# arnab39/Semi-supervised-segmentation-cycleGAN

Hardware: AMD Instinct MI355X
Metric: training images/sec (G+D step) at 256x256 (higher is better)
Workload: dtype f32; 1 GPU; VOC2012 21-class 256x256 semisupervised_cycleGAN as-written G+D step, batch=8 per GPU, fp32 tensors, 3-piece split-bf16 contraction, fp32-accurate (six exact bf16 piece products per fp32 product on the bf16 matrix cores, fp32 accumulation - forward, data and weight gradients; 21 / 20-channel stems and heads zero-padded onto the same contraction, 1- / 3-channel ends on the exact fp32 MFMA); global_batch=8, image_unit=one labeled + one unlabeled 256x256 image, parallelism=dp1, losses_finite=True

## Files before the change

semi-supervised-segmentation-cyclegan_amd/csrc/conv_wgrad.hip:

```cpp
#include "common.h"
#include <cstdlib>
#include "sscg_internal.h"

namespace {

constexpr int BKP = 32;

struct WgParams {
    const void* __restrict__ x;
    const void* __restrict__ dy;
    float* __restrict__ out;
    int Kc;
    int Ng;
    int C;
    int H, W, P, Q;
    int S;
    int stride, pad, dil, pad_mode;
    int npix;
    int chunk;
    int tiles_n;
    int tiles;
    int splits;
    float beta;
    FastDiv div_pq, div_q;
};

__device__ float sscg_zero_page[64];

template <int WM, int WN, int TM, int TN, int VA, int VB, bool DMA = false, int BF16 = 0, typename TX = float, typename TY = float>
__global__ __launch_bounds__(256) void conv_wgrad_kernel(WgParams p) {
    static_assert(!DMA || (VA == 4 && VB == 4), "LDS-DMA staging needs 16-byte granules");
    static_assert(!DMA || (sizeof(TX) == 4 && sizeof(TY) == 4), "LDS-DMA copies fp32 tiles");
    constexpr int BM = WM * TM * 32;
    constexpr int BN = WN * TN * 32;
    constexpr int LDA = DMA ? BM : BM + 4;
    constexpr int LDB = DMA ? BN : BN + 4;
    constexpr int CA = BM / VA;
    constexpr int CB = BN / VB;
    constexpr int RA = 256 / CA;
    constexpr int RB = 256 / CB;
    constexpr int PA = BKP / RA;
    constexpr int PB = BKP / RB;
    static_assert(256 % CA == 0 && 256 % CB == 0 && BKP % RA == 0 && BKP % RB == 0, "loader geometry");

    extern __shared__ __attribute__((aligned(16))) char smem_raw[];
    float* As = reinterpret_cast<float*>(smem_raw);
    float* Bs = As + 2 * BKP * LDA;

    const int tid = threadIdx.x;
    const int lin = xcd_remap(blockIdx.x, gridDim.x);
    const int split = lin / p.tiles;
    const int tl = lin - split * p.tiles;
    const int tile_n = tl % p.tiles_n;
    const int tile_m = tl / p.tiles_n;
    const int m0 = tile_m * BM;
    const int n0 = tile_n * BN;
    const int p_begin = split * p.chunk;
    const int p_end = min(p.npix, p_begin + p.chunk);

    const int ca = tid % CA, ra0 = tid / CA;
    const int ma = m0 + ca * VA;
    const bool a_col_ok = ma < p.Kc;
    const int cb = tid % CB, rb0 = tid / CB;
    const int nb = n0 + cb * VB;
    const bool b_col_ok = nb < p.Ng;
    int tdy = 0, tdx = 0, cch = 0;
    if (b_col_ok) {
        int tap = nb / p.C;
        cch = nb - tap * p.C;
        int ky = tap / p.S;
        int kx = tap - ky * p.S;
        tdy = ky * p.dil - p.pad;
        tdx = kx * p.dil - p.pad;
    }

    float ra[PA][VA];
    float rb[PB][VB];
    unsigned okmask = 0;

    const TY* dyc = reinterpret_cast<const TY*>(p.dy) + (a_col_ok ? ma : 0);
    const TX* xc = reinterpret_cast<const TX*>(p.x) + cch;
    const bool reflect = p.pad_mode == 1;

    int dma_buf = 0;
    const int wave_id = tid >> 6;
    auto load_tile = [&](int pt) {
        okmask = 0;
        if constexpr (DMA) {
            float* la = As + dma_buf * BKP * LDA + wave_id * 256;
            float* lb = Bs + dma_buf * BKP * LDB + wave_id * 256;
#pragma unroll
            for (int ps = 0; ps < PA; ++ps) {
                const int pix = pt + ra0 + ps * RA;
                const bool ok = a_col_ok && pix < p_end;
                const void* g = ok ? (const void*)(dyc + (size_t)pix * p.Kc) : (const void*)sscg_zero_page;
                __builtin_amdgcn_global_load_lds((const __attribute__((address_space(1))) void*)g,
                                                 (__attribute__((address_space(3))) void*)(la + ps * RA * LDA), 16, 0, 0);
            }
#pragma unroll
            for (int ps = 0; ps < PB; ++ps) {
                const int pix = pt + rb0 + ps * RB;
                bool ok = b_col_ok && pix < p_end;
                const int pp = ok ? pix : 0;
                const int img = fd_div(pp, p.div_pq);
                const int rem = pp - img * (p.P * p.Q);
                const int oy = fd_div(rem, p.div_q);
                const int ox = rem - oy * p.Q;
                int sy = oy * p.stride + tdy;
                int sx = ox * p.stride + tdx;
                int ry = sy < 0 ? -sy : sy;
                int rx = sx < 0 ? -sx : sx;
                ry = ry >= p.H ? 2 * (p.H - 1) - ry : ry;
                rx = rx >= p.W ? 2 * (p.W - 1) - rx : rx;
                sy = reflect ? ry : sy;
                sx = reflect ? rx : sx;
                ok = ok && ((unsigned)sy < (unsigned)p.H) && ((unsigned)sx < (unsigned)p.W);
                const void* g = ok ? (const void*)(xc + (size_t)((img * p.H + sy) * p.W + sx) * p.C) : (const void*)sscg_zero_page;
                __builtin_amdgcn_global_load_lds((const __attribute__((address_space(1))) void*)g,
                                                 (__attribute__((address_space(3))) void*)(lb + ps * RB * LDB), 16, 0, 0);
            }
            dma_buf ^= 1;
            return;
        }
#pragma unroll
        for (int ps = 0; ps < PA; ++ps) {
            const int pix = pt + ra0 + ps * RA;
            const bool ok = a_col_ok && pix < p_end;
            okmask |= ok ? (1u << ps) : 0u;
            const TY* g = dyc + (size_t)(ok ? pix : 0) * p.Kc;
            if constexpr (VA == 4) ld4<TY>(g, ra[ps]);
            else ra[ps][0] = ld1<TY>(g);
        }
#pragma unroll
        for (int ps = 0; ps < PB; ++ps) {
            const int pix = pt + rb0 + ps * RB;
            bool ok = b_col_ok && pix < p_end;
            const int pp = ok ? pix : 0;
            const int img = fd_div(pp, p.div_pq);
            const int rem = pp - img * (p.P * p.Q);
            const int oy = fd_div(rem, p.div_q);
            const int ox = rem - oy * p.Q;
            int sy = oy * p.stride + tdy;
            int sx = ox * p.stride + tdx;
            int ry = sy < 0 ? -sy : sy;
            int rx = sx < 0 ? -sx : sx;
            ry = ry >= p.H ? 2 * (p.H - 1) - ry : ry;
            rx = rx >= p.W ? 2 * (p.W - 1) - rx : rx;
            sy = reflect ? ry : sy;
            sx = reflect ? rx : sx;
            ok = ok && ((unsigned)sy < (unsigned)p.H) && ((unsigned)sx < (unsigned)p.W);
            okmask |= ok ? (1u << (16 + ps)) : 0u;
            const int spix = ok ? (img * p.H + sy) * p.W + sx : 0;
            const TX* g = xc + (size_t)spix * p.C;
            if constexpr (VB == 4) ld4<TX>(g, rb[ps]);
            else rb[ps][0] = ld1<TX>(g);
        }
    };

    auto store_tile = [&](int buf) {
        if constexpr (DMA) return;
        float* a = As + buf * BKP * LDA;
        float* b = Bs + buf * BKP * LDB;
#pragma unroll
        for (int ps = 0; ps < PA; ++ps) {
            float* d = a + (ra0 + ps * RA) * LDA + ca * VA;
            const bool ok = (okmask >> ps) & 1u;
            if constexpr (VA == 4) {
                f32x4 v;
#pragma unroll
                for (int e = 0; e < 4; ++e) v[e] = ok ? ra[ps][e] : 0.f;
                *reinterpret_cast<f32x4*>(d) = v;
            } else {
                *d = ok ? ra[ps][0] : 0.f;
            }
        }
#pragma unroll
        for (int ps = 0; ps < PB; ++ps) {
            float* d = b + (rb0 + ps * RB) * LDB + cb * VB;
            const bool ok = (okmask >> (16 + ps)) & 1u;
            if constexpr (VB == 4) {
                f32x4 v;
#pragma unroll
                for (int e = 0; e < 4; ++e) v[e] = ok ? rb[ps][e] : 0.f;
                *reinterpret_cast<f32x4*>(d) = v;
            } else {
                *d = ok ? rb[ps][0] : 0.f;
            }
        }
    };

    const int wave = tid >> 6;
    const int lane = tid & 63;
    const int li = lane & 31;
    const int lh = lane >> 5;
    const int wm = wave / WN;
    const int wn = wave % WN;
    const int row_w = wm * TM * 32;
    const int col_w = wn * TN * 32;

    f32x16 acc[TM][TN];
#pragma unroll
    for (int i = 0; i < TM; ++i)
#pragma unroll
        for (int j = 0; j < TN; ++j)
#pragma unroll
            for (int e = 0; e < 16; ++e) acc[i][j][e] = 0.f;

    const int nsteps = (p_end - p_begin + BKP - 1) / BKP;
    if (nsteps > 0) {
        load_tile(p_begin);
        store_tile(0);
    }
    __syncthreads();
    for (int it = 0; it < nsteps; ++it) {
        const int buf = it & 1;
        if (it + 1 < nsteps) load_tile(p_begin + (it + 1) * BKP);
        const float* a = As + buf * BKP * LDA + lh * LDA + row_w + li;
        const float* b = Bs + buf * BKP * LDB + lh * LDB + col_w + li;
        if constexpr (BF16) {
#pragma unroll
            for (int g2 = 0; g2 < BKP / 16; ++g2) {
                if constexpr (BF16 == 2) {
                    bf16x8 a0[TM], a1[TM], a2[TM], b0[TN], b1[TN], b2[TN];
#pragma unroll
                    for (int i = 0; i < TM; ++i) {
                        float v[8];
#pragma unroll
                        for (int e = 0; e < 8; ++e) v[e] = a[(g2 * 8 + e) * 2 * LDA + i * 32];
                        sscg_split8(v, a0[i], a1[i], a2[i]);
                    }
#pragma unroll
                    for (int j = 0; j < TN; ++j) {
                        float v[8];
#pragma unroll
                        for (int e = 0; e < 8; ++e) v[e] = b[(g2 * 8 + e) * 2 * LDB + j * 32];
                        sscg_split8(v, b0[j], b1[j], b2[j]);
                    }
#pragma unroll
                    for (int t = 0; t < 6; ++t)
#pragma unroll
                        for (int i = 0; i < TM; ++i)
#pragma unroll
                            for (int j = 0; j < TN; ++j) {
                                const bf16x8& pa = t == 0 ? a2[i] : (t == 1 || t == 3) ? a1[i] : a0[i];
                                const bf16x8& pb = (t == 0 || t == 3 || t == 5) ? b0[j] : (t == 1 || t == 4) ? b1[j] : b2[j];
                                acc[i][j] = __builtin_amdgcn_mfma_f32_32x32x16_bf16(pa, pb, acc[i][j], 0, 0, 0);
                            }
                    continue;
                }
                bf16x8 pa[TM], pb[TN];
#pragma unroll
                for (int e = 0; e < 8; ++e) {
                    const int kp = g2 * 8 + e;
#pragma unroll
                    for (int i = 0; i < TM; ++i) pa[i][e] = (__bf16)a[kp * 2 * LDA + i * 32];
#pragma unroll
                    for (int j = 0; j < TN; ++j) pb[j][e] = (__bf16)b[kp * 2 * LDB + j * 32];
                }
#pragma unroll
                for (int i = 0; i < TM; ++i)
#pragma unroll
                    for (int j = 0; j < TN; ++j)
                        acc[i][j] = __builtin_amdgcn_mfma_f32_32x32x16_bf16(pa[i], pb[j], acc[i][j], 0, 0, 0);
            }
        } else {
#pragma unroll
        for (int kp = 0; kp < BKP / 2; ++kp) {
            float fa[TM], fb[TN];
#pragma unroll
            for (int i = 0; i < TM; ++i) fa[i] = a[kp * 2 * LDA + i * 32];
#pragma unroll
            for (int j = 0; j < TN; ++j) fb[j] = b[kp * 2 * LDB + j * 32];
#pragma unroll
            for (int i = 0; i < TM; ++i)
#pragma unroll
                for (int j = 0; j < TN; ++j)
                    acc[i][j] = __builtin_amdgcn_mfma_f32_32x32x2f32(fa[i], fb[j], acc[i][j], 0, 0, 0);
        }
        }
        if (it + 1 < nsteps) store_tile(buf ^ 1);
        __syncthreads();
    }

    float* out = p.out + (size_t)split * p.Kc * p.Ng;
    const bool direct = (p.splits == 1);
    if constexpr (VB == 4) {
        sscg_stage_store_tile<BM, BN, 256, TM, TN>(acc, reinterpret_cast<float*>(smem_raw), out, m0, n0, p.Kc, p.Ng, row_w, col_w, li, lh, tid,
                                                   direct ? p.beta : 0.f);
        return;
    }
#pragma unroll
    for (int j = 0; j < TN; ++j) {
        const int n = n0 + col_w + j * 32 + li;
        if (n >= p.Ng) continue;
#pragma unroll
        for (int i = 0; i < TM; ++i) {
#pragma unroll
            for (int e = 0; e < 16; ++e) {
                const int m = m0 + row_w + i * 32 + (e & 3) + 8 * (e >> 2) + 4 * lh;
                if (m < p.Kc) {
                    size_t o = (size_t)m * p.Ng + n;
                    float v = acc[i][j][e];
                    if (direct && p.beta != 0.f) v += p.beta * out[o];
                    out[o] = v;
                }
            }
        }
    }
}

template <int V>
__global__ __launch_bounds__(256) void wgrad_reduce_kernel(const float* __restrict__ ws, float* __restrict__ dw, size_t n, int splits,
                                                            float beta) {
    const size_t i = ((size_t)blockIdx.x * blockDim.x + threadIdx.x) * V;
    if (i >= n) return;
    typedef float vec_t __attribute__((ext_vector_type(V)));
    vec_t s = 0.f;
#pragma unroll 16
    for (int k = 0; k < splits; ++k) s += *reinterpret_cast<const vec_t*>(ws + (size_t)k * n + i);
    vec_t* d = reinterpret_cast<vec_t*>(dw + i);
    *d = (beta != 0.f) ? beta * *d + s : s;
}

__global__ __launch_bounds__(256) void wgrad_reduce_w4_kernel(const float* __restrict__ ws, float* __restrict__ dw, size_t n, int splits,
                                                               float beta) {
    __shared__ f32x4 sm[3][64];
    const int v = threadIdx.x & 63, sl = threadIdx.x >> 6;
    const size_t i = ((size_t)blockIdx.x * 64 + v) * 4;
    f32x4 s = 0.f;
    if (i < n) {
#pragma unroll 8
        for (int k = sl; k < splits; k += 4) s += *reinterpret_cast<const f32x4*>(ws + (size_t)k * n + i);
    }
    if (sl) sm[sl - 1][v] = s;
    __syncthreads();
    if (sl == 0 && i < n) {
        s = ((s + sm[0][v]) + sm[1][v]) + sm[2][v];
        f32x4* d = reinterpret_cast<f32x4*>(dw + i);
        *d = (beta != 0.f) ? beta * *d + s : s;
    }
}

struct WgPlan {
    int cfg;
    int bm, bn;
    int splits;
    int chunk;
};


struct WgClass { int cfg, bm, bn; float t_step_us, c0; float f[4]; };
const WgClass WG_CLASSES[] = {
    {0, 128, 128, 2.13f, 1.5f, {1.25f, 1.f, 1.f, 1.f}},
    {1, 64, 64, 0.59f, 2.f, {1.5f, 1.17f, 1.08f, 1.f}},
    {2, 32, 128, 0.70f, 2.f, {1.5f, 1.17f, 1.08f, 1.f}},
    {3, 128, 32, 0.70f, 2.f, {1.5f, 1.17f, 1.08f, 1.f}},
};

float wgrad_cost_us(const WgClass& c, long tiles, long steps, long s, double out_bytes) {
    long r = cdiv(tiles * s, 256);
    float f = c.f[r > 4 ? 3 : r - 1];
    float t = (float)r * ((float)cdiv(steps, s) + c.c0) * c.t_step_us * f;
    if (s > 1) t += (float)(2.0 * s * out_bytes / 4.0e6) + 4.f;
    return t;
}

WgPlan plan_wgrad(const sscg_conv_desc* d) {
    WgPlan pl;
    const int Kc = d->K;
    const int Ng = d->R * d->S * d->C;
    const long npix = (long)d->N * d->P * d->Q;
    const long steps = cdiv(npix, BKP);
    const double out_bytes = (double)Kc * Ng * sizeof(float);
    int first = 0, last = 1;
    if (d->precision == 2 && Kc >= 128 && Ng >= 128) last = 0;
    if (Kc <= 32) first = last = 2;
    else if (Ng <= 32 || d->C < 32) first = last = 3;
    else if (Kc <= 64 || Ng <= 64) first = last = 1;
    float best = 0.f;
    long best_s = 1;
    pl.cfg = -1;
    for (int ci = first; ci <= last; ++ci) {
        const WgClass& c = WG_CLASSES[ci];
        const long tiles = (long)cdiv(Kc, c.bm) * cdiv(Ng, c.bn);
        const long smax = steps / 2 < 1 ? 1 : (steps / 2 > 512 ? 512 : steps / 2);
        long prev = 0;
        for (int k = 0; k <= 16; ++k) {
            long sp = k == 0 ? 1 : (256L * k) / tiles;
            if (sp < 1) sp = 1;
            if (sp > smax) sp = smax;
            if (sp == prev) continue;
            prev = sp;
            float t = wgrad_cost_us(c, tiles, steps, sp, out_bytes);
            if (pl.cfg < 0 || t < best) { best = t; best_s = sp; pl.cfg = c.cfg; pl.bm = c.bm; pl.bn = c.bn; }
        }
    }
    long splits = best_s;
    const int force_cfg = (d->wgrad_tuning & 0xff) - 1, force_splits = (d->wgrad_tuning >> 8) & 0xffff;
    if (force_cfg >= 0 && force_cfg <= 1 && force_splits > 0 && pl.cfg <= 1) {
        pl.cfg = force_cfg;
        pl.bm = pl.bn = pl.cfg == 0 ? 128 : 64;
        splits = force_splits;
        if (splits > steps) splits = steps;
    }
    long steps_per = cdiv(steps, splits);
    pl.chunk = (int)(steps_per * BKP);
    pl.splits = cdiv(npix, pl.chunk);
    return pl;
}

template <int WM, int WN, int TM, int TN, int VA, int VB, bool DMA = false, int BF16 = 0, typename TX = float, typename TY = float>
int launch_wg(WgParams p, int splits, hipStream_t st) {
    constexpr int BM = WM * TM * 32;
    constexpr int BN = WN * TN * 32;
    p.tiles_n = cdiv(p.Ng, BN);
    int tiles_m = cdiv(p.Kc, BM);
    p.tiles = tiles_m * p.tiles_n;
    p.splits = splits;
    size_t smem = (size_t)(2 * BKP * (DMA ? BM : BM + 4) + 2 * BKP * (DMA ? BN : BN + 4)) * sizeof(float);
    if (VB == 4 && smem < (size_t)BM * (BN + 4) * sizeof(float)) smem = (size_t)BM * (BN + 4) * sizeof(float);
    auto kern = conv_wgrad_kernel<WM, WN, TM, TN, VA, VB, DMA, BF16, TX, TY>;
    SSCG_ENSURE_SMEM((kern), smem);
    hipLaunchKernelGGL(kern, dim3(p.tiles * splits), dim3(256), smem, st, p);
    SSCG_LAUNCH_CHECK();
    return SSCG_OK;
}

template <int VA, int VB>
int dispatch_wg(const WgParams& p, const WgPlan& pl, int precision, hipStream_t st) {
    switch (pl.cfg) {
        case 0: if (precision == 1) return launch_wg<2, 2, 2, 2, VA, VB, (VA == 4 && VB == 4), 1>(p, pl.splits, st);
                if constexpr (VA == 4 && VB == 4) { if (precision == 2) return launch_wg<2, 2, 2, 2, VA, VB, true, 2>(p, pl.splits, st); }
                return launch_wg<2, 2, 2, 2, VA, VB, (VA == 4 && VB == 4)>(p, pl.splits, st);
        case 1: if (precision == 1) return launch_wg<2, 2, 1, 1, VA, VB, (VA == 4 && VB == 4), 1>(p, pl.splits, st);
                if constexpr (VA == 4 && VB == 4) { if (precision == 2) return launch_wg<2, 2, 1, 1, VA, VB, true, 2>(p, pl.splits, st); }
                return launch_wg<2, 2, 1, 1, VA, VB, (VA == 4 && VB == 4)>(p, pl.splits, st);
        case 2: if (precision == 1) return launch_wg<1, 4, 1, 1, VA, VB, false, true>(p, pl.splits, st);
                return launch_wg<1, 4, 1, 1, VA, VB>(p, pl.splits, st);
        case 3: if (precision == 1) return launch_wg<4, 1, 1, 1, VA, VB, false, true>(p, pl.splits, st);
                return launch_wg<4, 1, 1, 1, VA, VB>(p, pl.splits, st);
        default: return SSCG_ERR_BAD_ARG;
    }
}

template <int VA, int VB, typename TX, typename TY>
int dispatch_wg_mixed(const WgParams& p, const WgPlan& pl, hipStream_t st) {
    switch (pl.cfg) {
        case 2: return launch_wg<1, 4, 1, 1, VA, VB, false, true, TX, TY>(p, pl.splits, st);
        case 3: return launch_wg<4, 1, 1, 1, VA, VB, false, true, TX, TY>(p, pl.splits, st);
        default: return SSCG_ERR_UNSUPPORTED;
    }
}

template <typename TX, typename TY>
int dispatch_wg_types(const WgParams& p, const WgPlan& pl, bool va4, bool vb4, hipStream_t st) {
    if (va4 && vb4) return dispatch_wg_mixed<4, 4, TX, TY>(p, pl, st);
    if (va4) return dispatch_wg_mixed<4, 1, TX, TY>(p, pl, st);
    if (vb4) return dispatch_wg_mixed<1, 4, TX, TY>(p, pl, st);
    return dispatch_wg_mixed<1, 1, TX, TY>(p, pl, st);
}

}

namespace {

constexpr int THIN_MAX = 32;
constexpr int THIN_BLOCKS = 1024;

struct ThinParams {
    const void* __restrict__ wide;
    const void* __restrict__ thin;
    float* __restrict__ part;
    int npix, Wd, T;
};

template <int T, typename TW, typename TT>
__global__ __launch_bounds__(256) void thin_wgrad_kernel(ThinParams p) {
    const TW* wide = reinterpret_cast<const TW*>(p.wide);
    const TT* thin = reinterpret_cast<const TT*>(p.thin);
    constexpr int TB = T < 4 ? T : 4;
    extern __shared__ float red[];
    const int wq = p.Wd / 4;
    const int lanes = 256 / wq;
    const int q = threadIdx.x % wq;
    const int pl = threadIdx.x / wq;
    float acc[T][4];
#pragma unroll
    for (int t = 0; t < T; ++t)
#pragma unroll
        for (int e = 0; e < 4; ++e) acc[t][e] = 0.f;
    if (pl < lanes) {
        const int stride = lanes * gridDim.x;
        int px = blockIdx.x * lanes + pl;
        for (; px + stride < p.npix; px += 2 * stride) {
            float w0[4], w1[4];
            ld4<TW>(wide + (size_t)px * p.Wd + q * 4, w0);
            ld4<TW>(wide + (size_t)(px + stride) * p.Wd + q * 4, w1);
            const TT* th0 = thin + (size_t)px * T;
            const TT* th1 = thin + (size_t)(px + stride) * T;
#pragma unroll
            for (int t = 0; t < T; ++t) {
                const float v0 = ld1<TT>(th0 + t), v1 = ld1<TT>(th1 + t);
#pragma unroll
                for (int e = 0; e < 4; ++e) acc[t][e] = fmaf(v1, w1[e], fmaf(v0, w0[e], acc[t][e]));
            }
        }
        if (px < p.npix) {
            float w0[4];
            ld4<TW>(wide + (size_t)px * p.Wd + q * 4, w0);
            const TT* th0 = thin + (size_t)px * T;
#pragma unroll
            for (int t = 0; t < T; ++t) {
                const float v0 = ld1<TT>(th0 + t);
#pragma unroll
                for (int e = 0; e < 4; ++e) acc[t][e] = fmaf(v0, w0[e], acc[t][e]);
            }
        }
    }
#pragma unroll
    for (int t0 = 0; t0 < T; t0 += TB) {
        if (pl < lanes) {
#pragma unroll
            for (int t = 0; t < TB; ++t)
                if (t0 + t < T)
#pragma unroll
                    for (int e = 0; e < 4; ++e) red[((size_t)pl * TB + t) * p.Wd + q * 4 + e] = acc[t0 + t][e];
        }
        __syncthreads();
        const int nt = (T - t0) < TB ? (T - t0) : TB;
        for (int i = threadIdx.x; i < nt * p.Wd; i += 256) {
            float s = 0.f;
            for (int l = 0; l < lanes; ++l) s += red[(size_t)l * TB * p.Wd + i];
            p.part[(size_t)blockIdx.x * T * p.Wd + (size_t)t0 * p.Wd + i] = s;
        }
        __syncthreads();
    }
}

__global__ __launch_bounds__(256) void thin_wgrad_reduce_kernel(const float* __restrict__ part, float* __restrict__ dw, int blocks,
                                                                 int T, int Wd, int K, int C, float beta) {
    const int o = blockIdx.x * 4 + (threadIdx.x >> 6);
    const int lane = threadIdx.x & 63;
    if (o >= T * Wd) return;
    float s = 0.f;
    for (int b = lane; b < blocks; b += 64) s += part[(size_t)b * T * Wd + o];
    s = wave_sum(s);
    if (lane == 0) {
        const int t = o / Wd, w = o - t * Wd;
        const int k = (K == T && K <= C) ? t : w;
        const int c = (K == T && K <= C) ? w : t;
        float* d = dw + (size_t)k * C + c;
        *d = beta != 0.f ? beta * *d + s : s;
    }
}

bool thin_wgrad_applies(const sscg_conv_desc* d) {
    if (d->R != 1 || d->S != 1 || d->stride != 1 || d->pad != 0 || d->pad_mode != 0) return false;
    const int T = d->K < d->C ? d->K : d->C, Wd = d->K < d->C ? d->C : d->K;
    return T <= THIN_MAX && Wd % 4 == 0 && Wd <= 256 && Wd >= 16 && (long)d->N * d->H * d->W >= 65536;
}

template <int T, typename TW, typename TT>
int launch_thin(const ThinParams& p, int blocks, size_t smem, hipStream_t st) {
    SSCG_ENSURE_SMEM((thin_wgrad_kernel<T, TW, TT>), smem);
    hipLaunchKernelGGL((thin_wgrad_kernel<T, TW, TT>), dim3(blocks), dim3(256), smem, st, p);
    return SSCG_OK;
}

template <typename TW, typename TT>
int launch_thin_T(const ThinParams& p, size_t smem, hipStream_t st) {
    switch (p.T) {
        case 1: return launch_thin<1, TW, TT>(p, THIN_BLOCKS, smem, st);
        case 2: return launch_thin<2, TW, TT>(p, THIN_BLOCKS, smem, st);
        case 3: return launch_thin<3, TW, TT>(p, THIN_BLOCKS, smem, st);
        case 4: return launch_thin<4, TW, TT>(p, THIN_BLOCKS, smem, st);
        case 20: return launch_thin<20, TW, TT>(p, THIN_BLOCKS, smem, st);
        case 21: return launch_thin<21, TW, TT>(p, THIN_BLOCKS, smem, st);
        default: return SSCG_ERR_UNSUPPORTED;
    }
}

int thin_wgrad(const sscg_conv_desc* d, const void* x, const void* dy, float* dw, float beta, void* ws, hipStream_t st) {
    const bool thin_is_k = d->K <= d->C;
    ThinParams p;
    p.T = thin_is_k ? d->K : d->C;
    p.Wd = thin_is_k ? d->C : d->K;
    p.wide = thin_is_k ? x : dy;
    p.thin = thin_is_k ? dy : x;
    const int wide_dt = thin_is_k ? d->x_dtype : d->y_dtype, thin_dt = thin_is_k ? d->y_dtype : d->x_dtype;
    p.part = reinterpret_cast<float*>(ws);
    p.npix = d->N * d->H * d->W;
    const int lanes = 256 / (p.Wd / 4);
    const size_t smem = (size_t)lanes * (p.T < 4 ? p.T : 4) * p.Wd * sizeof(float);
    int rc;
    if (wide_dt == SSCG_F32 && thin_dt == SSCG_F32) rc = launch_thin_T<float, float>(p, smem, st);
    else if (wide_dt == SSCG_BF16 && thin_dt == SSCG_F32) rc = launch_thin_T<__bf16, float>(p, smem, st);
    else if (wide_dt == SSCG_BF16 && thin_dt == SSCG_BF16) rc = launch_thin_T<__bf16, __bf16>(p, smem, st);
    else rc = SSCG_ERR_UNSUPPORTED;
    if (rc) return rc;
    SSCG_LAUNCH_CHECK();
    hipLaunchKernelGGL(thin_wgrad_reduce_kernel, dim3(cdiv(p.T * p.Wd, 4)), dim3(256), 0, st, p.part, dw, THIN_BLOCKS, p.T, p.Wd,
                       d->K, d->C, beta);
    SSCG_LAUNCH_CHECK();
    return SSCG_OK;
}

bool thin_wgrad_supported_T(int T) { return T == 1 || T == 2 || T == 3 || T == 4 || T == 20 || T == 21; }

}

int sscg_wgrad_reduce(const float* ws, float* dw, size_t n, int splits, float beta, hipStream_t st) {
    static const bool w4 = !(getenv("SSCG_WGRAD_REDUCE_W4") && atoi(getenv("SSCG_WGRAD_REDUCE_W4")) == 0);
    const bool vec_ok = n % 4 == 0 && ((size_t)dw & 15) == 0 && ((size_t)ws & 15) == 0;
    if (vec_ok && w4 && splits >= 8 && n / 4 <= 64 * 16384)
        hipLaunchKernelGGL(wgrad_reduce_w4_kernel, dim3(cdiv((long)(n / 4), 64)), dim3(256), 0, st, ws, dw, n, splits, beta);
    else if (vec_ok)
        hipLaunchKernelGGL(wgrad_reduce_kernel<4>, dim3(cdiv((long)(n / 4), 256)), dim3(256), 0, st, ws, dw, n, splits, beta);
    else
        hipLaunchKernelGGL(wgrad_reduce_kernel<1>, dim3(cdiv((long)n, 256)), dim3(256), 0, st, ws, dw, n, splits, beta);
    SSCG_LAUNCH_CHECK();
    return SSCG_OK;
}

static bool wg_dt_ok(int dt) { return dt == SSCG_F32 || dt == SSCG_BF16; }

extern "C" size_t sscg_conv2d_wgrad_workspace(const sscg_conv_desc* d) {
    if (!d) return 0;
    if (thin_wgrad_applies(d) && thin_wgrad_supported_T(d->K < d->C ? d->K : d->C))
        return (size_t)THIN_BLOCKS * d->K * d->C * sizeof(float);
    if (sscg_wgrad16_applies(d)) return sscg_wgrad16_workspace(d);
    if (sscg_wgrads_applies(d)) return sscg_wgrads_workspace(d);
    WgPlan pl = plan_wgrad(d);
    if (pl.splits <= 1) return 0;
    return (size_t)pl.splits * d->K * d->R * d->S * d->C * sizeof(float);
}

extern "C" int sscg_conv2d_wgrad(const sscg_conv_desc* d, const void* x, const void* dy, float* dw, float beta,
                                 void* ws, size_t ws_bytes, void* stream) {
    if (!d || !x || !dy || !dw) return SSCG_ERR_BAD_ARG;
    if (d->N <= 0 || d->C <= 0 || d->K <= 0 || !wg_dt_ok(d->x_dtype) || !wg_dt_ok(d->y_dtype)) return SSCG_ERR_BAD_ARG;
    if ((long)d->N * d->H * d->W * (long)d->C >= (1L << 31)) return SSCG_ERR_UNSUPPORTED;
    if ((long)d->N * d->P * d->Q * (long)d->K >= (1L << 31)) return SSCG_ERR_UNSUPPORTED;
    hipStream_t st = (hipStream_t)stream;
    if (thin_wgrad_applies(d) && thin_wgrad_supported_T(d->K < d->C ? d->K : d->C)) {
        if (!ws || ws_bytes < sscg_conv2d_wgrad_workspace(d)) return SSCG_ERR_WORKSPACE;
        return thin_wgrad(d, x, dy, dw, beta, ws, st);
    }
    if (sscg_wgrad16_applies(d)) return sscg_wgrad16(d, x, dy, dw, beta, ws, ws_bytes, st);
    if (sscg_wgrads_applies(d)) return sscg_wgrads(d, x, dy, dw, beta, ws, ws_bytes, st);
    WgPlan pl = plan_wgrad(d);
    size_t need = pl.splits > 1 ? (size_t)pl.splits * d->K * d->R * d->S * d->C * sizeof(float) : 0;
    if (need > 0 && (!ws || ws_bytes < need)) return SSCG_ERR_WORKSPACE;
    WgParams p;
    p.x = x; p.dy = dy;
    p.out = pl.splits > 1 ? reinterpret_cast<float*>(ws) : dw;
    p.Kc = d->K; p.Ng = d->R * d->S * d->C; p.C = d->C;
    p.H = d->H; p.W = d->W; p.P = d->P; p.Q = d->Q; p.S = d->S;
    p.stride = d->stride; p.pad = d->pad; p.dil = d->dil; p.pad_mode = d->pad_mode;
    p.npix = d->N * d->P * d->Q; p.chunk = pl.chunk; p.tiles_n = 0; p.tiles = 0; p.splits = 1;
    p.beta = pl.splits > 1 ? 0.f : beta;
    p.div_pq = make_fastdiv(d->P * d->Q);
    p.div_q = make_fastdiv(d->Q);
    const bool va4 = (d->K % 4 == 0), vb4 = (d->C % 4 == 0);
    int rc;
    if (d->x_dtype == SSCG_F32 && d->y_dtype == SSCG_F32) {
        if (va4 && vb4) rc = dispatch_wg<4, 4>(p, pl, d->precision, st);
        else if (va4) rc = dispatch_wg<4, 1>(p, pl, d->precision, st);
        else if (vb4) rc = dispatch_wg<1, 4>(p, pl, d->precision, st);
        else rc = dispatch_wg<1, 1>(p, pl, d->precision, st);
    } else if (d->x_dtype == SSCG_F32) {
        rc = dispatch_wg_types<float, __bf16>(p, pl, va4, vb4, st);
    } else if (d->y_dtype == SSCG_F32) {
        rc = dispatch_wg_types<__bf16, float>(p, pl, va4, vb4, st);
    } else {
        rc = SSCG_ERR_UNSUPPORTED;
    }
    if (rc) return rc;
    if (pl.splits > 1) return sscg_wgrad_reduce(reinterpret_cast<const float*>(ws), dw, (size_t)d->K * p.Ng, pl.splits, beta, st);
    return SSCG_OK;
}
```

Measured before the change: 65.24 img/s.

## Add dedicated weight-gradient paths for thin and ragged-channel conv ends

```diff
diff --git a/semi-supervised-segmentation-cyclegan_amd/csrc/conv_wgrad.hip b/semi-supervised-segmentation-cyclegan_amd/csrc/conv_wgrad.hip
--- a/semi-supervised-segmentation-cyclegan_amd/csrc/conv_wgrad.hip
+++ b/semi-supervised-segmentation-cyclegan_amd/csrc/conv_wgrad.hip
@@ -427,7 +427,10 @@
 }
 
 template <int VA, int VB>
-int dispatch_wg(const WgParams& p, const WgPlan& pl, int precision, hipStream_t st) {
+int dispatch_wg(const WgParams& p, const WgPlan& pl, int precision, hipStream_t st, bool split_small = false) {
+    if constexpr (VA == 4 && VB == 4) {
+        if (split_small && precision == 2 && pl.cfg == 2) return launch_wg<1, 4, 1, 1, 4, 4, true, 2>(p, pl.splits, st);
+    }
     switch (pl.cfg) {
         case 0: if (precision == 1) return launch_wg<2, 2, 2, 2, VA, VB, (VA == 4 && VB == 4), 1>(p, pl.splits, st);
                 if constexpr (VA == 4 && VB == 4) { if (precision == 2) return launch_wg<2, 2, 2, 2, VA, VB, true, 2>(p, pl.splits, st); }
@@ -609,6 +612,175 @@
 
 }
 
+int sscg_wgrad_reduce(const float* ws, float* dw, size_t n, int splits, float beta, hipStream_t st);
+
+namespace {
+
+__global__ __launch_bounds__(256) void wgrad_reduce_cut_kernel(const float* __restrict__ ws, float* __restrict__ dw, size_t n_out, int C, int Cp,
+                                                                size_t split_stride, int splits, float beta) {
+    const size_t i = (size_t)blockIdx.x * 256 + threadIdx.x;
+    if (i >= n_out) return;
+    const size_t row = i / C;
+    const size_t src = row * Cp + (i - row * C);
+    float s = 0.f;
+#pragma unroll 8
+    for (int k = 0; k < splits; ++k) s += ws[(size_t)k * split_stride + src];
+    dw[i] = (beta != 0.f) ? beta * dw[i] + s : s;
+}
+
+constexpr int TT_SLAB = 256;
+constexpr int TT_MAXK = 3;
+
+struct ThinTapsParams {
+    const float* __restrict__ x;
+    const float* __restrict__ dy;
+    float* __restrict__ part;
+    int npix;
+    int H, W, C, P, Q, pad, dil;
+    int ppb;
+    FastDiv div_hw, div_w;
+};
+
+template <int T, int R, int S>
+__global__ __launch_bounds__(256) void thin_taps_wgrad_kernel(ThinTapsParams p) {
+    constexpr int TAPS = R * S;
+    __shared__ float red[4][TAPS][TT_SLAB];
+    const int lane = threadIdx.x & 63;
+    const int wv = __builtin_amdgcn_readfirstlane(threadIdx.x >> 6);
+    const int c0 = blockIdx.x * TT_SLAB + lane * 4;
+    const bool c_ok = c0 < p.C;
+    const int p0 = blockIdx.y * p.ppb;
+    const int p1 = min(p.npix, p0 + p.ppb);
+    float acc[T][TAPS][4];
+#pragma unroll
+    for (int t = 0; t < T; ++t)
+#pragma unroll
+        for (int k = 0; k < TAPS; ++k)
+#pragma unroll
+            for (int e = 0; e < 4; ++e) acc[t][k][e] = 0.f;
+    const float* xc = p.x + (c_ok ? c0 : 0);
+    f32x4 cur = 0.f;
+    int px = p0 + wv;
+    if (px < p1 && c_ok) cur = *reinterpret_cast<const f32x4*>(xc + (size_t)px * p.C);
+    for (; px < p1; px += 4) {
+        f32x4 nxt = 0.f;
+        if (px + 4 < p1 && c_ok) nxt = *reinterpret_cast<const f32x4*>(xc + (size_t)(px + 4) * p.C);
+        const int img = fd_div(px, p.div_hw);
+        const int rem = px - img * (p.H * p.W);
+        const int iy = fd_div(rem, p.div_w);
+        const int ix = rem - iy * p.W;
+#pragma unroll
+        for (int ky = 0; ky < R; ++ky) {
+            const int oy = iy + p.pad - ky * p.dil;
+            if ((unsigned)oy >= (unsigned)p.P) continue;
+#pragma unroll
+            for (int kx = 0; kx < S; ++kx) {
+                const int ox = ix + p.pad - kx * p.dil;
+                if ((unsigned)ox >= (unsigned)p.Q) continue;
+                const float* g = p.dy + (size_t)((img * p.P + oy) * p.Q + ox) * T;
+#pragma unroll
+                for (int t = 0; t < T; ++t) {
+                    const float v = g[t];
+#pragma unroll
+                    for (int e = 0; e < 4; ++e) acc[t][ky * S + kx][e] = fmaf(v, cur[e], acc[t][ky * S + kx][e]);
+                }
+            }
+        }
+        cur = nxt;
+    }
+#pragma unroll
+    for (int t = 0; t < T; ++t) {
+#pragma unroll
+        for (int k = 0; k < TAPS; ++k)
+            *reinterpret_cast<f32x4*>(&red[wv][k][lane * 4]) = f32x4{acc[t][k][0], acc[t][k][1], acc[t][k][2], acc[t][k][3]};
+        __syncthreads();
+        const int c = blockIdx.x * TT_SLAB + threadIdx.x;
+        if (c < p.C) {
+            float* o = p.part + ((size_t)blockIdx.y * T + t) * TAPS * p.C + c;
+#pragma unroll
+            for (int k = 0; k < TAPS; ++k)
+                o[(size_t)k * p.C] = ((red[0][k][threadIdx.x] + red[1][k][threadIdx.x]) + red[2][k][threadIdx.x]) + red[3][k][threadIdx.x];
+        }
+        __syncthreads();
+    }
+}
+
+struct EndsPlan {
+    int kind;
+    int Cp, Kp;
+    WgPlan pl;
+    size_t pad_bytes;
+    int ppb, pblocks;
+    size_t ws_bytes;
+};
+
+EndsPlan plan_ends(const sscg_conv_desc* d) {
+    static const bool on = !(getenv("SSCG_WGRAD_THIN_ENDS") && atoi(getenv("SSCG_WGRAD_THIN_ENDS")) == 0);
+    EndsPlan e;
+    e.kind = 0; e.Cp = d->C; e.Kp = d->K; e.pad_bytes = 0; e.ppb = 0; e.pblocks = 0; e.ws_bytes = 0;
+    if (!on || d->precision != 2 || d->x_dtype != SSCG_F32 || d->y_dtype != SSCG_F32 || d->pad_mode != 0) return e;
+    const int taps = d->R * d->S;
+    if (d->K <= TT_MAXK && d->R == 3 && d->S == 3 && d->stride == 1 && d->C % 4 == 0 && d->C >= 64) {
+        const int npix = d->N * d->H * d->W;
+        const int slabs = cdiv(d->C, TT_SLAB);
+        int pb = cdiv(512, slabs);
+        if (pb > cdiv(npix, 8)) pb = cdiv(npix, 8);
+        e.ppb = cdiv(cdiv(npix, pb), 4) * 4;
+        e.pblocks = cdiv(npix, e.ppb);
+        e.kind = 2;
+        e.ws_bytes = (size_t)e.pblocks * d->K * taps * d->C * sizeof(float);
+        return e;
+    }
+    const bool ragged_c = d->C % 4 != 0 && d->K % 4 == 0 && d->K >= 32 && (d->C < 4 || (d->C > 16 && d->C < 32));
+    const bool ragged_k = d->K % 4 != 0 && d->C % 4 == 0 && d->C >= 32 && d->K > 16 && d->K < 32;
+    if (!ragged_c && !ragged_k) return e;
+    if (ragged_c) e.Cp = d->C < 4 ? 4 : 32;
+    if (ragged_k) e.Kp = 32;
+    sscg_conv_desc t = *d;
+    t.C = e.Cp; t.K = e.Kp;
+    if (sscg_wgrads_applies(&t)) return e;
+    const long npix = (long)d->N * d->P * d->Q;
+    const long steps = cdiv(npix, BKP);
+    if (steps < 2) return e;
+    e.pl = plan_wgrad(&t);
+    if (e.pl.splits < 2) {
+        e.pl.chunk = (int)(cdiv(steps, 2) * BKP);
+        e.pl.splits = cdiv(npix, e.pl.chunk);
+    }
+    const size_t rows = ragged_c ? (size_t)d->N * d->H * d->W : (size_t)npix;
+    e.pad_bytes = (rows * (ragged_c ? e.Cp : e.Kp) * sizeof(float) + 255) & ~(size_t)255;
+    e.ws_bytes = e.pad_bytes + (size_t)e.pl.splits * e.Kp * taps * e.Cp * sizeof(float);
+    e.kind = 1;
+    return e;
+}
+
+template <int T>
+int launch_thin_taps(const ThinTapsParams& p, dim3 grid, hipStream_t st) {
+    hipLaunchKernelGGL((thin_taps_wgrad_kernel<T, 3, 3>), grid, dim3(256), 0, st, p);
+    SSCG_LAUNCH_CHECK();
+    return SSCG_OK;
+}
+
+int thin_taps_wgrad(const sscg_conv_desc* d, const EndsPlan& e, const void* x, const void* dy, float* dw, float beta, void* ws, hipStream_t st) {
+    ThinTapsParams p;
+    p.x = reinterpret_cast<const float*>(x); p.dy = reinterpret_cast<const float*>(dy); p.part = reinterpret_cast<float*>(ws);
+    p.npix = d->N * d->H * d->W; p.H = d->H; p.W = d->W; p.C = d->C; p.P = d->P; p.Q = d->Q; p.pad = d->pad; p.dil = d->dil;
+    p.ppb = e.ppb;
+    p.div_hw = make_fastdiv(d->H * d->W);
+    p.div_w = make_fastdiv(d->W);
+    const dim3 grid(cdiv(d->C, TT_SLAB), e.pblocks);
+    int rc;
+    switch (d->K) {
+        case 1: rc = launch_thin_taps<1>(p, grid, st); break;
+        case 2: rc = launch_thin_taps<2>(p, grid, st); break;
+        default: rc = launch_thin_taps<3>(p, grid, st); break;
+    }
+    if (rc) return rc;
+    return sscg_wgrad_reduce(p.part, dw, (size_t)d->K * d->R * d->S * d->C, e.pblocks, beta, st);
+}
+
+}
+
 int sscg_wgrad_reduce(const float* ws, float* dw, size_t n, int splits, float beta, hipStream_t st) {
     static const bool w4 = !(getenv("SSCG_WGRAD_REDUCE_W4") && atoi(getenv("SSCG_WGRAD_REDUCE_W4")) == 0);
     const bool vec_ok = n % 4 == 0 && ((size_t)dw & 15) == 0 && ((size_t)ws & 15) == 0;
@@ -622,6 +794,54 @@
     return SSCG_OK;
 }
 
+static int wg_launch(const sscg_conv_desc* d, const WgPlan& pl, const void* x, const void* dy, float* out, float beta, bool split_small,
+                     hipStream_t st) {
+    WgParams p;
+    p.x = x; p.dy = dy;
+    p.out = out;
+    p.Kc = d->K; p.Ng = d->R * d->S * d->C; p.C = d->C;
+    p.H = d->H; p.W = d->W; p.P = d->P; p.Q = d->Q; p.S = d->S;
+    p.stride = d->stride; p.pad = d->pad; p.dil = d->dil; p.pad_mode = d->pad_mode;
+    p.npix = d->N * d->P * d->Q; p.chunk = pl.chunk; p.tiles_n = 0; p.tiles = 0; p.splits = 1;
+    p.beta = pl.splits > 1 ? 0.f : beta;
+    p.div_pq = make_fastdiv(d->P * d->Q);
+    p.div_q = make_fastdiv(d->Q);
+    const bool va4 = (d->K % 4 == 0), vb4 = (d->C % 4 == 0);
+    if (d->x_dtype == SSCG_F32 && d->y_dtype == SSCG_F32) {
+        if (va4 && vb4) return dispatch_wg<4, 4>(p, pl, d->precision, st, split_small);
+        if (va4) return dispatch_wg<4, 1>(p, pl, d->precision, st);
+        if (vb4) return dispatch_wg<1, 4>(p, pl, d->precision, st);
+        return dispatch_wg<1, 1>(p, pl, d->precision, st);
+    }
+    if (d->x_dtype == SSCG_F32) return dispatch_wg_types<float, __bf16>(p, pl, va4, vb4, st);
+    if (d->y_dtype == SSCG_F32) return dispatch_wg_types<__bf16, float>(p, pl, va4, vb4, st);
+    return SSCG_ERR_UNSUPPORTED;
+}
+
+static int padded_ends_wgrad(const sscg_conv_desc* d, const EndsPlan& e, const void* x, const void* dy, float* dw, float beta, void* ws,
+                             hipStream_t st) {
+    float* padded = reinterpret_cast<float*>(ws);
+    float* part = reinterpret_cast<float*>(reinterpret_cast<char*>(ws) + e.pad_bytes);
+    sscg_conv_desc t = *d;
+    t.C = e.Cp; t.K = e.Kp;
+    int rc;
+    if (e.Cp != d->C) {
+        rc = sscg_resize_channels(reinterpret_cast<const float*>(x), padded, (int64_t)d->N * d->H * d->W, d->C, e.Cp, st);
+        x = padded;
+    } else {
+        rc = sscg_resize_channels(reinterpret_cast<const float*>(dy), padded, (int64_t)d->N * d->P * d->Q, d->K, e.Kp, st);
+        dy = padded;
+    }
+    if (rc) return rc;
+    rc = wg_launch(&t, e.pl, x, dy, part, 0.f, true, st);
+    if (rc) return rc;
+    const size_t n_out = (size_t)d->K * d->R * d->S * d->C;
+    hipLaunchKernelGGL(wgrad_reduce_cut_kernel, dim3((unsigned)cdiv((long)n_out, 256)), dim3(256), 0, st, part, dw, n_out, d->C, e.Cp,
+                       (size_t)e.Kp * d->R * d->S * e.Cp, e.pl.splits, beta);
+    SSCG_LAUNCH_CHECK();
+    return SSCG_OK;
+}
+
 static bool wg_dt_ok(int dt) { return dt == SSCG_F32 || dt == SSCG_BF16; }
 
 extern "C" size_t sscg_conv2d_wgrad_workspace(const sscg_conv_desc* d) {
@@ -630,6 +850,8 @@
         return (size_t)THIN_BLOCKS * d->K * d->C * sizeof(float);
     if (sscg_wgrad16_applies(d)) return sscg_wgrad16_workspace(d);
     if (sscg_wgrads_applies(d)) return sscg_wgrads_workspace(d);
+    const EndsPlan e = plan_ends(d);
+    if (e.kind) return e.ws_bytes;
     WgPlan pl = plan_wgrad(d);
     if (pl.splits <= 1) return 0;
     return (size_t)pl.splits * d->K * d->R * d->S * d->C * sizeof(float);
@@ -648,34 +870,17 @@
     }
     if (sscg_wgrad16_applies(d)) return sscg_wgrad16(d, x, dy, dw, beta, ws, ws_bytes, st);
     if (sscg_wgrads_applies(d)) return sscg_wgrads(d, x, dy, dw, beta, ws, ws_bytes, st);
+    const EndsPlan e = plan_ends(d);
+    if (e.kind) {
+        if (!ws || ws_bytes < e.ws_bytes) return SSCG_ERR_WORKSPACE;
+        if (e.kind == 2) return thin_taps_wgrad(d, e, x, dy, dw, beta, ws, st);
+        return padded_ends_wgrad(d, e, x, dy, dw, beta, ws, st);
+    }
     WgPlan pl = plan_wgrad(d);
     size_t need = pl.splits > 1 ? (size_t)pl.splits * d->K * d->R * d->S * d->C * sizeof(float) : 0;
     if (need > 0 && (!ws || ws_bytes < need)) return SSCG_ERR_WORKSPACE;
-    WgParams p;
-    p.x = x; p.dy = dy;
-    p.out = pl.splits > 1 ? reinterpret_cast<float*>(ws) : dw;
-    p.Kc = d->K; p.Ng = d->R * d->S * d->C; p.C = d->C;
-    p.H = d->H; p.W = d->W; p.P = d->P; p.Q = d->Q; p.S = d->S;
-    p.stride = d->stride; p.pad = d->pad; p.dil = d->dil; p.pad_mode = d->pad_mode;
-    p.npix = d->N * d->P * d->Q; p.chunk = pl.chunk; p.tiles_n = 0; p.tiles = 0; p.splits = 1;
-    p.beta = pl.splits > 1 ? 0.f : beta;
-    p.div_pq = make_fastdiv(d->P * d->Q);
-    p.div_q = make_fastdiv(d->Q);
-    const bool va4 = (d->K % 4 == 0), vb4 = (d->C % 4 == 0);
-    int rc;
-    if (d->x_dtype == SSCG_F32 && d->y_dtype == SSCG_F32) {
-        if (va4 && vb4) rc = dispatch_wg<4, 4>(p, pl, d->precision, st);
-        else if (va4) rc = dispatch_wg<4, 1>(p, pl, d->precision, st);
-        else if (vb4) rc = dispatch_wg<1, 4>(p, pl, d->precision, st);
-        else rc = dispatch_wg<1, 1>(p, pl, d->precision, st);
-    } else if (d->x_dtype == SSCG_F32) {
-        rc = dispatch_wg_types<float, __bf16>(p, pl, va4, vb4, st);
-    } else if (d->y_dtype == SSCG_F32) {
-        rc = dispatch_wg_types<__bf16, float>(p, pl, va4, vb4, st);
-    } else {
-        rc = SSCG_ERR_UNSUPPORTED;
-    }
+    int rc = wg_launch(d, pl, x, dy, pl.splits > 1 ? reinterpret_cast<float*>(ws) : dw, beta, false, st);
     if (rc) return rc;
-    if (pl.splits > 1) return sscg_wgrad_reduce(reinterpret_cast<const float*>(ws), dw, (size_t)d->K * p.Ng, pl.splits, beta, st);
+    if (pl.splits > 1) return sscg_wgrad_reduce(reinterpret_cast<const float*>(ws), dw, (size_t)d->K * d->R * d->S * d->C, pl.splits, beta, st);
     return SSCG_OK;
 }
```

Result: slower. 60.06 img/s (-7.9%).
